# ThibHlln/smartpy

Hardware: AMD Instinct MI355X
Metric: MC sample-timesteps/sec/GPU; 1e5 LHS x hourly 10-yr forcing (higher is better)
Workload: dtype f64

## Files before the change

smartpy_amd/csrc/smart_capi.hip:

```cpp
#include "smart_capi_internal.h"
#include "smart_fast_entry.h"

#include <cmath>
#include <cstdarg>
#include <cstdio>
#include <cstdlib>
#include <cstring>
#include <mutex>
#include <vector>

namespace smart {

static_assert(kStatusSliceTimeout == SMART_STATUS_SLICE_TIMEOUT && kStatusStalePlan == SMART_STATUS_STALE_PLAN,
              "status bits of smart_device.h and include/smart_amd.h");

static thread_local char g_err[512] = "";

int fail(int code, const char *fmt, ...)
{
    va_list ap;
    va_start(ap, fmt);
    vsnprintf(g_err, sizeof(g_err), fmt, ap);
    va_end(ap);
    return code;
}

void clear_error() { g_err[0] = 0; }

int hip_fail(hipError_t e, const char *what) { return fail(SMART_E_NO_DEVICE, "%s: %s", what, hipGetErrorString(e)); }

__global__ __launch_bounds__(256) void smart_obs_prepare(const double *obs, long R, double *ws)
{
    __shared__ double sh[512];
    __shared__ double st[5];
    const long c = blockIdx.x;
    double *w = ws + c * (kWsHead + R);
    obs_stats<true>(obs + c * R, R, st, w + kWsHead, sh);
    const long r1 = first_observed_row(obs + c * R, R, sh);
    if (threadIdx.x < 5)
        w[threadIdx.x] = st[threadIdx.x];
    if (threadIdx.x == 5)
        w[kWsFirst] = (double)r1;
}

__global__ void smart_forcing_scan(KArgs a, const double2 *__restrict__ forcing)
{
    const double2 *__restrict__ f = forcing + (long)blockIdx.y * a.T;
    int bad = 0;
    bool wild = false;
    const unsigned long long top = 0x7ff0000000000000ull;
    for (long t = (long)blockIdx.x * blockDim.x + threadIdx.x; t < a.T; t += (long)gridDim.x * blockDim.x) {
        bad |= forcing_flags_of_step(a, f, t);
        const double2 v = f[t];
        wild = wild || (__builtin_bit_cast(unsigned long long, v.x) & top) == top ||
               (__builtin_bit_cast(unsigned long long, v.y) & top) == top;
    }
    if (a.codes) {
        uint2 *codes = const_cast<uint2 *>(a.codes) + (long)blockIdx.y * code_chunks(a.T);
        for (long ch = (long)blockIdx.x * blockDim.x + threadIdx.x; ch < code_chunks(a.T);
             ch += (long)gridDim.x * blockDim.x) {
            uint2 w = make_uint2(0u, 0u);
            if ((ch + 1) * kChunk <= a.T) {
                const double2 *__restrict__ v = f + ch * kChunk;
                w = chunk_codes(ch, step_kind(v[0]), step_kind(v[1]), step_kind(v[2]), step_kind(v[3]), a.pair_stride);
            }
            codes[ch] = w;
        }
    }
    if (a.estream) {
        double *rec = const_cast<double *>(a.estream) + (long)blockIdx.y * every_pairs(a.T) * 8;
        unsigned *codes = const_cast<unsigned *>(a.ecodes) + (long)blockIdx.y * every_pairs(a.T);
        const double *obs = a.obs ? a.obs + (long)blockIdx.y * a.R : nullptr;
        const double *dev = a.ws ? a.ws + (long)blockIdx.y * (kWsHead + a.R) + kWsHead : nullptr;
        for (long p = (long)blockIdx.x * blockDim.x + threadIdx.x; p < every_pairs(a.T); p += (long)gridDim.x * blockDim.x) {
            double r[8] = {0.0, 0.0, 0.0, 0.0, 0.0, 0.0, 0.0, 0.0};
            unsigned code = 0;
            if (2 * p + 1 < a.T) {
                for (int j = 0; j < 2; ++j) {
                    const long t = 2 * p + j, rr = (t + 1) % a.gap == 0 ? (t + 1) / a.gap - 1 : -1;
                    r[4 * j] = f[t].x;
                    r[4 * j + 1] = f[t].y;
                    r[4 * j + 2] = obs && dev && rr >= 0 && rr < a.R ? obs[rr] : 0.0;
                    r[4 * j + 3] = obs && dev && rr >= 0 && rr < a.R ? dev[rr] : 0.0;
                }
                code = a.gap == 1 ? every_code(p, step_kind(f[2 * p]), step_kind(f[2 * p + 1]))
                                  : gap_code(p, a.gap, step_kind(f[2 * p]), step_kind(f[2 * p + 1]));
            }
            for (int j = 0; j < 8; ++j)
                rec[p * 8 + j] = r[j];
            codes[p] = code;
        }
    }
    if (bad)
        __hip_atomic_fetch_or(a.fflags + blockIdx.y, bad, __ATOMIC_RELAXED, __HIP_MEMORY_SCOPE_AGENT);
    if (wild && a.hdr)
        __hip_atomic_fetch_or(a.hdr + kHdrStatus, kStatusNonFiniteForcing, __ATOMIC_RELAXED, __HIP_MEMORY_SCOPE_AGENT);
}

__global__ void smart_workspace_reset(int *hdr, long n_hdr, int *flags, long n_flags)
{
    const long i = (long)blockIdx.x * blockDim.x + threadIdx.x;
    if (i < n_hdr)
        hdr[i] = 0;
    if (i < n_flags)
        flags[i] = 0;
}

__global__ __launch_bounds__(kWave) void smart_classify_rows(KArgs a)
{
    const int cls = wave_class(a, (long)blockIdx.x, (long)blockIdx.y);
    if (threadIdx.x == 0) {
        __hip_atomic_fetch_or(a.hdr + kHdrPlan, 1 << cls, __ATOMIC_RELAXED, __HIP_MEMORY_SCOPE_AGENT);
        if (cls == 3)
            __hip_atomic_fetch_add(a.hdr + kHdrPlanIllCond, 1, __ATOMIC_RELAXED, __HIP_MEMORY_SCOPE_AGENT);
    }
}

__global__ void smart_classify_forcing(KArgs a, int *hdr)
{
    const long c = (long)blockIdx.x * blockDim.x + threadIdx.x;
    if (c < a.n_catch) {
        const int kind = forcing_kind(a, a.fflags[c]);
        __hip_atomic_fetch_or(hdr + kHdrPlan,
                              kind == kForcingIntervals ? SMART_PLAN_FORCING_PIECEWISE
                                                        : (kind == kForcingRuns ? SMART_PLAN_FORCING_RUNS
                                                                                : SMART_PLAN_FORCING_VARYING),
                              __ATOMIC_RELAXED, __HIP_MEMORY_SCOPE_AGENT);
    }
}

constexpr int kMaxDevices = 64, kMaxTodo = 8, kMaxAux = kMaxTodo - 1;

struct DeviceCtx {
    std::once_flag once;
    int n_simd = 0;
    std::mutex mu;
    hipStream_t aux[kMaxAux] = {};
    hipEvent_t fork = nullptr, join[kMaxAux] = {};
    size_t lds_size[kNumFastKernels][17] = {};
    bool lds_known[kNumFastKernels][17] = {};
};

static DeviceCtx g_dev[kMaxDevices];

static DeviceCtx *device_ctx()
{
    int dev = 0;
    if (hipGetDevice(&dev) != hipSuccess || dev < 0 || dev >= kMaxDevices)
        return nullptr;
    DeviceCtx *d = &g_dev[dev];
    std::call_once(d->once, [d, dev] {
        int cus = 0;
        if (hipDeviceGetAttribute(&cus, hipDeviceAttributeMultiprocessorCount, dev) == hipSuccess && cus > 0)
            d->n_simd = cus * 4;
    });
    return d->n_simd > 0 ? d : nullptr;
}

struct Overrides {
    int pair_blocks = -1;
    int time_slices = 0;
    int illcond_form = SMART_LITERAL_FORM_AUTO;
    int exits = -1;
    long max_polls = kDefaultMaxPolls;
    int drop_slice = 0;
    bool allsteps_fast = false;
};

static Overrides read_overrides()
{
    Overrides o;
    if (const char *v = getenv("SMART_PAIR_BLOCKS"))
        o.pair_blocks = atoi(v) != 0;
    if (const char *v = getenv("SMART_TIME_SLICES"))
        o.time_slices = atoi(v) <= 0 ? 1 : atoi(v);
    if (const char *v = getenv("SMART_ILLCOND_FORM"))
        o.illcond_form = !strcmp(v, "rows")    ? SMART_LITERAL_FORM_ROWS
                         : !strcmp(v, "lanes") ? SMART_LITERAL_FORM_LANES
                                               : SMART_LITERAL_FORM_AUTO;
    if (const char *v = getenv("SMART_EXITS"))
        o.exits = atoi(v) != 0;
    if (const char *v = getenv("SMART_DEBUG_MAX_POLLS"))
        o.max_polls = atol(v) > 0 ? atol(v) : kDefaultMaxPolls;
    if (const char *v = getenv("SMART_DEBUG_DROP_SLICE"))
        o.drop_slice = atoi(v);
    if (const char *v = getenv("SMART_ALLSTEPS_MATH"))
        o.allsteps_fast = !strcmp(v, "fast");
    return o;
}

struct FastKernelInfo {
    const void *handle;
    const char *name;
    int cls;
    bool sliced;
    int waves;
};

static const FastKernelInfo kFastKernels[kNumFastKernels] = {
#define X(id, symbol, cls, sliced, waves) {reinterpret_cast<const void *>(&symbol), #symbol, cls, sliced, waves},
    SMART_FAST_KERNELS(X)
#undef X
};

static size_t lds_for_residency(DeviceCtx *d, FastKernel k, int per_cu)
{
    if (per_cu < 1 || per_cu > 16)
        return 0;
    if (!d->lds_known[k][per_cu]) {
        size_t found = 0;
        for (size_t x = (size_t)(160 * 1024 / per_cu) / 256 * 256;
             x >= 1024 && x > (size_t)(160 * 1024 / (per_cu + 1)) - 2048; x -= 256) {
            int nb = 0;
            if (hipOccupancyMaxActiveBlocksPerMultiprocessor(&nb, kFastKernels[k].handle, kWave, x) != hipSuccess)
                break;
            if (nb == per_cu) {
                found = x;
                break;
            }
            if (nb > per_cu)
                break;
        }
        d->lds_size[k][per_cu] = found;
        d->lds_known[k][per_cu] = true;
    }
    return d->lds_size[k][per_cu];
}

static int merged_report(const SmartEnsemble *e);

extern "C" __attribute__((used, visibility("default"))) volatile char smart_lint_stamp[40] = "SMART_LINT_STAMP=unchecked";

static bool pair_blocks_wanted(const Overrides &ov)
{
    if (ov.pair_blocks >= 0)
        return ov.pair_blocks != 0;
    static const char ok[] = "SMART_LINT_STAMP=pairs-ok";
    for (size_t i = 0; i + 1 < sizeof(ok); ++i)
        if (smart_lint_stamp[i] != ok[i])
            return false;
    return true;
}

static bool uses_records(const SmartEnsemble *e)
{
    const int merged = merged_report(e);
    return merged == kReportEvery || ((merged == kReportMean || merged == kReportLast) && e->report_gap % kChunk != 0);
}

struct Layout {
    size_t header = 0;
    size_t stats_off = 0, stats = 0;
    size_t state_off = 0, state = 0;
    size_t flags_off = 0, flags = 0;
    size_t codes_off = 0, codes = 0;
    size_t ecodes_off = 0;
    size_t total = 0;
    size_t handover() const { return state + flags; }
};

static bool sizes_make_sense(const SmartEnsemble *e)
{
    return e->n_catchments >= 1 && e->n_samples >= 1 && e->n_steps >= 0 && e->report_gap >= 1;
}

static Layout layout(const SmartEnsemble *e, bool sliced)
{
    Layout l;
    const size_t C = (size_t)(e->n_catchments < 1 ? 1 : e->n_catchments);
    l.header = ((size_t)kHdrInts + C) * sizeof(int);
    l.header = (l.header + 255) / 256 * 256;
    if (!sizes_make_sense(e))
        return l;
    l.stats_off = l.header;
    if (e->objfn)
        l.stats = C * (size_t)(kWsHead + smart_n_reports(e->n_steps, e->report_gap, e->report_type)) * sizeof(double);
    l.state_off = l.stats_off + l.stats;
    const size_t blocks = (size_t)((e->n_samples + kWave - 1) / kWave) * C;
    if (sliced) {
        l.state = blocks * kSegFields * kWave * sizeof(double);
        l.flags = (blocks + 1) / 2 * 2 * sizeof(int);
    }
    l.flags_off = l.state_off + l.state;
    l.codes_off = l.ecodes_off = l.flags_off + l.flags;
    const int merged = merged_report(e);
    if (e->math_mode != SMART_MATH_FAST) {
    } else if (uses_records(e)) {
        const size_t records = C * (size_t)every_pairs(e->n_steps) * 8 * sizeof(double);
        l.ecodes_off = l.codes_off + records;
        l.codes = records + C * (size_t)every_pairs(e->n_steps) * sizeof(unsigned);
    } else if (merged == kReportMean || merged == kReportLast) {
        l.codes = C * (size_t)code_chunks(e->n_steps) * sizeof(uint2);
    }
    l.codes = (l.codes + 255) / 256 * 256;
    l.total = l.codes_off + l.codes;
    return l;
}

static int check(const SmartEnsemble *e)
{
    if (!e)
        return fail(SMART_E_NULL, "SmartEnsemble pointer is NULL");
    if (e->n_catchments < 1 || e->n_samples < 1 || e->n_steps < 1 || e->n_warm < 0 || e->report_gap < 1)
        return fail(SMART_E_SIZE, "sizes must satisfy n_catchments, n_samples, n_steps, report_gap >= 1 and n_warm >= 0 "
                                  "(got %lld, %lld, %lld, %lld, %lld)",
                    (long long)e->n_catchments, (long long)e->n_samples, (long long)e->n_steps,
                    (long long)e->report_gap, (long long)e->n_warm);
    if (e->report_type != SMART_REPORT_SUMMARY && e->report_type != SMART_REPORT_RAW)
        return fail(SMART_E_REPORT_TYPE, "Reporting type '%d' unknown.", (int)e->report_type);
    if (e->math_mode != SMART_MATH_LITERAL && e->math_mode != SMART_MATH_FAST)
        return fail(SMART_E_MODE, "math mode '%d' unknown.", (int)e->math_mode);
    if (e->n_warm > e->n_steps)
        return fail(SMART_E_WARMUP, "The warm-up duration (%lld steps) cannot exceed the length of the simulation period "
                                    "(%lld steps) because the beginning of the simulation period is used as made-up "
                                    "warm-up data.",
                    (long long)e->n_warm, (long long)e->n_steps);
    if (e->report_type == SMART_REPORT_SUMMARY && (e->n_steps % e->report_gap || e->n_warm % e->report_gap))
        return fail(SMART_E_GAP, "summary report: simulation length %lld and warm-up length %lld must be multiples of the "
                                 "report gap %lld",
                    (long long)e->n_steps, (long long)e->n_warm, (long long)e->report_gap);
    if (!(e->delta_sec > 0.0))
        return fail(SMART_E_SIZE, "delta_sec must be > 0");
    if (!e->area_m2 || !e->forcing || !e->params || !e->gw)
        return fail(SMART_E_NULL, "area_m2, forcing, params and gw are required");
    if (e->params_catchment_stride != 0 && e->params_catchment_stride < e->n_samples * 10)
        return fail(SMART_E_SIZE, "params_catchment_stride must be 0 or >= n_samples * 10");
    if (e->discharge && e->discharge_ld < e->n_samples)
        return fail(SMART_E_SIZE, "discharge_ld must be >= n_samples");
    if (e->objfn && (!e->obs || !e->workspace))
        return fail(SMART_E_NULL, "objfn needs obs and workspace");
    if (e->objfn && e->workspace_bytes < (int64_t)layout(e, false).state_off)
        return fail(SMART_E_SIZE, "workspace_bytes %lld is less than the %lld the header and the observation statistics need",
                    (long long)e->workspace_bytes, (long long)layout(e, false).state_off);
    if (e->time_slices < 0)
        return fail(SMART_E_SIZE, "time_slices must be >= 0");
    if (e->plan != 0 && !(e->plan & SMART_PLAN_VALID))
        return fail(SMART_E_SIZE, "plan must be 0 or a value returned by smart_plan_ensemble");
    if (e->literal_form < SMART_LITERAL_FORM_AUTO || e->literal_form > SMART_LITERAL_FORM_LANES)
        return fail(SMART_E_MODE, "literal_form must be SMART_LITERAL_FORM_AUTO, _ROWS or _LANES");
    clear_error();
    return SMART_OK;
}

int device_ready()
{
    int n = 0;
    hipError_t err = hipGetDeviceCount(&n);
    if (err != hipSuccess)
        return hip_fail(err, "hipGetDeviceCount");
    if (n < 1)
        return fail(SMART_E_NO_DEVICE, "no HIP device is visible; this engine has no CPU fallback");
    return SMART_OK;
}

static int merged_report(const SmartEnsemble *e)
{
    if (e->report_type == SMART_REPORT_SUMMARY && e->report_gap >= 2)
        return kReportMean;
    if (e->final_vars)
        return -1;
    if (e->report_gap == 1)
        return kReportEvery;
    if (e->report_type == SMART_REPORT_RAW && e->n_steps % e->report_gap == 0 && e->n_warm % e->report_gap == 0)
        return kReportLast;
    return -1;
}

static int plan_time_slices(const SmartEnsemble *e, int n_simd, const Overrides &ov, int *per_simd, double *load)
{
    const long blocks = (e->n_samples + kWave - 1) / kWave * e->n_catchments;
    const long cap = (blocks + n_simd - 1) / n_simd;
    *per_simd = (int)(cap < 1 ? 1 : cap);
    *load = (double)blocks / (double)n_simd;
    if (merged_report(e) < 0)
        return 1;
    const long n_all = e->n_warm / e->report_gap + e->n_steps / e->report_gap;
    const int forced = e->time_slices ? e->time_slices : ov.time_slices;
    if (forced == 1 || n_all < 64)
        return 1;
    if (forced > 1)
        return forced < n_all / 4 ? forced : (int)(n_all / 4);
    if (blocks <= n_simd || blocks > 48L * n_simd)
        return 1;
    const long want = blocks >= 10L * n_simd ? 8 : 24;
    return (int)(n_all / 64 < want ? n_all / 64 : want);
}

static bool device_says_sliced(const SmartEnsemble *e, const Overrides &ov)
{
    if (e->math_mode != SMART_MATH_FAST || !sizes_make_sense(e))
        return false;
    int per_simd = 0, n_dev = 0;
    double load = 0.0;
    DeviceCtx *d = hipGetDeviceCount(&n_dev) == hipSuccess && n_dev > 0 ? device_ctx() : nullptr;
    return d && plan_time_slices(e, d->n_simd, ov, &per_simd, &load) > 1;
}

struct Workspace {
    Layout lay;
    int *hdr = nullptr, *fflags = nullptr;
    double *stats = nullptr;
    char *state = nullptr;
    char *codes = nullptr;
};

static Workspace carve(const SmartEnsemble *e, const Overrides &ov)
{
    Workspace w;
    const Layout &l = w.lay = layout(e, device_says_sliced(e, ov));
    const size_t bytes = e->workspace && e->workspace_bytes > 0 ? (size_t)e->workspace_bytes : 0;
    if (bytes < l.header)
        return w;
    char *base = (char *)e->workspace;
    w.hdr = (int *)base;
    w.fflags = w.hdr + kHdrInts;
    if (l.stats && bytes >= l.state_off)
        w.stats = (double *)(base + l.stats_off);
    if (l.handover() && bytes >= l.codes_off)
        w.state = base + l.state_off;
    if (l.codes && bytes >= l.total)
        w.codes = base + l.codes_off;
    return w;
}

static KArgs kernel_args(const SmartEnsemble *e, const Workspace &w)
{
    KArgs a;
    a.N = e->n_samples;
    a.T = e->n_steps;
    a.W = e->n_warm;
    a.gap = e->report_gap;
    a.R = smart_n_reports(e->n_steps, e->report_gap, e->report_type);
    a.first_len = e->report_type == SMART_REPORT_RAW && e->n_steps % e->report_gap ? e->n_steps % e->report_gap
                                                                                 : e->report_gap;
    a.report_type = e->report_type;
    a.dt = e->delta_sec;
    a.area = e->area_m2;
    a.forcing = e->forcing;
    a.params = e->params;
    a.pstride_c = e->params_catchment_stride;
    a.extra = e->extra;
    a.initial = e->initial;
    a.obs = e->obs;
    a.gw_obs = e->gw_obs;
    a.ws = e->objfn ? w.stats : nullptr;
    a.discharge = e->discharge;
    a.ld = e->discharge_ld;
    a.gw = e->gw;
    a.objfn = e->objfn;
    a.final_vars = e->final_vars;
    a.np_mean = e->math_mode == SMART_MATH_LITERAL && e->report_type == SMART_REPORT_SUMMARY && a.gap >= 8 && a.gap <= 128;
    a.pair_stride = e->final_vars ? (int)kPairStrideSplit : (int)kPairStride;
    a.n_catch = e->n_catchments;
    a.n_blocks = (a.N + kWave - 1) / kWave;
    a.seg_blocks = a.n_blocks * a.n_catch;
    a.hdr = w.hdr;
    a.fflags = nullptr;
    const int merged = merged_report(e);
    if ((merged == kReportMean || merged == kReportLast) && a.gap <= 0x7fffffff) {
        for (long q = 1; q * q <= a.gap && a.n_div < kMaxDiv; ++q)
            if (a.gap % q == 0 && a.gap / q >= 2)
                a.div[a.n_div++] = (int)(a.gap / q);
        for (long q = (long)std::sqrt((double)a.gap) + 1; q >= 2 && a.n_div < kMaxDiv; --q)
            if (q * q < a.gap && a.gap % q == 0 && q < a.div[a.n_div - 1])
                a.div[a.n_div++] = (int)q;
    }
    return a;
}

static void reset_workspace(const Workspace &w, long n_catch, int *flags, long n_flags, hipStream_t s)
{
    const long n_hdr = kHdrInts + n_catch, n = n_hdr > n_flags ? n_hdr : n_flags;
    hipLaunchKernelGGL(smart_workspace_reset, dim3((unsigned)((n + 255) / 256)), dim3(256), 0, s, w.hdr, n_hdr, flags,
                       n_flags);
}

static void set_codes(KArgs *a, const Workspace &w, const Overrides &ov)
{
    a->codes = nullptr, a->estream = nullptr, a->ecodes = nullptr;
    if (!w.codes || !pair_blocks_wanted(ov))
        return;
    if (w.lay.ecodes_off != w.lay.codes_off) {
        a->estream = (const double *)w.codes;
        a->ecodes = (const unsigned *)(w.codes + (w.lay.ecodes_off - w.lay.codes_off));
    } else {
        a->codes = (const uint2 *)w.codes;
    }
}

static void scan_forcing(const SmartEnsemble *e, KArgs a, const Workspace &w, const Overrides &ov, hipStream_t s)
{
    a.fflags = w.fflags;
    set_codes(&a, w, ov);
    hipLaunchKernelGGL(smart_forcing_scan, dim3(64, (unsigned)e->n_catchments), dim3(256), 0, s, a,
                       reinterpret_cast<const double2 *>(e->forcing));
}

static hipError_t launch_kernel(FastKernel k, KArgs a, dim3 grid, size_t lds, hipStream_t s)
{
    const double2 *forcing = reinterpret_cast<const double2 *>(a.forcing);
    const double *obs = a.obs, *ws = a.ws;
    void *args[] = {&a, &forcing, &obs, &ws};
    return hipLaunchKernel(kFastKernels[k].handle, grid, dim3(kWave), args, lds, s);
}

struct Decision {
    FastKernel todo[kMaxTodo];
    int n_todo = 0;
    bool overflow = false;
    void push(FastKernel k)
    {
        if (n_todo < kMaxTodo)
            todo[n_todo++] = k;
        else
            overflow = true;
    }
    int n_seg = 1, per_simd = 0, exits = 0;
    int class_mask = 0, pc_mask = 0;
    int report = -1;
    bool intervals = false;
    double load = 0.0;
    long illcond_blocks = 0;
    bool illcond_rows = true;
};

constexpr int kIllCondRowRounds = 2;

static long count_illcond_blocks(const SmartEnsemble *e, int plan)
{
    const long counted = (plan >> SMART_PLAN_ILLCOND_BLOCKS_SHIFT) & SMART_PLAN_ILLCOND_BLOCKS_MAX;
    const long all = (long)((e->n_samples + kWave - 1) / kWave * e->n_catchments);
    return counted > 0 && counted < SMART_PLAN_ILLCOND_BLOCKS_MAX ? counted : all;
}

static bool illcond_form(const SmartEnsemble *e, int n_simd, long blocks, const Overrides &ov)
{
    const int form = e->literal_form != SMART_LITERAL_FORM_AUTO ? e->literal_form : ov.illcond_form;
    if (form != SMART_LITERAL_FORM_AUTO)
        return form == SMART_LITERAL_FORM_ROWS;
    const long all = (long)((e->n_samples + kWave - 1) / kWave * e->n_catchments);
    return blocks * kIllCondWaves + (all - blocks) <= (long)kIllCondRowRounds * n_simd;
}

static int decide(const SmartEnsemble *e, const DeviceCtx *d, const Workspace &w, const Overrides &ov, Decision *out)
{
    Decision &x = *out;
    x.report = merged_report(e);
    x.intervals = x.report == kReportMean;
    const int plan = (e->plan & SMART_PLAN_VALID) ? e->plan : (0x3f | SMART_PLAN_FORCING_RUNS);
    x.n_seg = plan_time_slices(e, d->n_simd, ov, &x.per_simd, &x.load);
    if (x.n_seg > 1 && !w.state)
        x.n_seg = 1;
    x.exits = ov.exits >= 0 ? ov.exits : x.load > 2.5;
    x.class_mask = plan & 0xf;
    if (plan & SMART_PLAN_CLASS_REGULAR) {
        if (x.intervals) {
            if (plan & SMART_PLAN_FORCING_PIECEWISE) {
                x.push(e->final_vars ? kIntervalsStates : (x.exits ? kIntervalsExits : kIntervals));
                x.pc_mask |= kPcIntervals;
            }
            if (plan & SMART_PLAN_FORCING_RUNS) {
                x.push(e->final_vars ? kRunsStates : (x.exits ? kRunsExits : kRuns));
                x.pc_mask |= kPcRuns;
            }
            if (plan & SMART_PLAN_FORCING_VARYING) {
                x.push(e->final_vars ? kStepsStates : kSteps);
                x.pc_mask |= kPcSteps;
            }
        } else if (x.report == kReportLast) {
            if (plan & SMART_PLAN_FORCING_PIECEWISE) {
                x.push(kIntervalsRaw);
                x.pc_mask |= kPcIntervals;
            }
            if (plan & (SMART_PLAN_FORCING_RUNS | SMART_PLAN_FORCING_VARYING)) {
                x.push(kStepsRaw);
                x.pc_mask |= kPcSteps | kPcRuns;
            }
        } else if (x.report == kReportEvery) {
            x.push(kStepsEvery);
            x.pc_mask = kPcIntervals | kPcSteps | kPcRuns;
        } else {
            x.push(kPlain);
        }
    }
    if (plan & SMART_PLAN_CLASS_STIFF)
        x.push(kStiff);
    if (plan & SMART_PLAN_CLASS_GUARD)
        x.push(kGuard);
    if (plan & SMART_PLAN_CLASS_ILLCOND) {
        x.illcond_blocks = count_illcond_blocks(e, plan);
        x.illcond_rows = illcond_form(e, d->n_simd, x.illcond_blocks, ov);
        x.push(x.illcond_rows ? kIllCond : kIllCondLanes);
    }
    if (x.overflow)
        return fail(SMART_E_SIZE, "internal: a call wants more than %d kernels", kMaxTodo);
    if (x.n_todo == 0)
        return fail(SMART_E_SIZE, "the plan names no class of rows");
    return SMART_OK;
}

static int run(const SmartEnsemble *e, const Overrides &ov, bool literal_rows = false)
{
    int rc = check(e);
    if (rc)
        return rc;
    if ((rc = device_ready()))
        return rc;
    hipStream_t s = (hipStream_t)e->stream;
    const Workspace w = carve(e, ov);
    KArgs a = kernel_args(e, w);

    if (e->objfn)
        hipLaunchKernelGGL(smart_obs_prepare, dim3((unsigned)e->n_catchments), dim3(256), 0, s, e->obs, a.R, w.stats);

    const dim3 grid((unsigned)a.n_blocks, (unsigned)e->n_catchments);
    if (e->math_mode == SMART_MATH_LITERAL) {
        if (w.hdr)
            reset_workspace(w, e->n_catchments, nullptr, 0, s);
        a.hdr = nullptr;
        launch_literal(a, grid, a.np_mean ? (size_t)a.gap * kWave * sizeof(double) : 0, s, literal_rows);
        HIP_TRY(hipGetLastError());
        return SMART_OK;
    }

    DeviceCtx *d = device_ctx();
    if (!d)
        return fail(SMART_E_NO_DEVICE, "cannot query the current HIP device");
    Decision x;
    if ((rc = decide(e, d, w, ov, &x)))
        return rc;
    const int n_seg = x.n_seg, n_todo = x.n_todo;
    a.exits = x.exits;
    a.class_mask = x.class_mask;
    a.pc_mask = x.pc_mask;

    KArgs a_sliced = a;
    if (n_seg > 1) {
        a_sliced.n_seg = n_seg;
        a_sliced.seg_state = (double *)w.state;
        a_sliced.seg_flag = (int *)(w.state + (w.lay.flags_off - w.lay.state_off));
        a_sliced.max_polls = ov.max_polls;
        a_sliced.debug_drop = ov.drop_slice;
    }
    if (w.hdr) {
        reset_workspace(w, e->n_catchments, a_sliced.seg_flag, n_seg > 1 ? a.seg_blocks : 0, s);
        scan_forcing(e, a, w, ov, s);
        if (x.report >= 0 && (x.class_mask & SMART_PLAN_CLASS_REGULAR)) {
            a.fflags = a_sliced.fflags = w.fflags;
            set_codes(&a, w, ov);
            a_sliced.codes = a.codes, a_sliced.estream = a.estream, a_sliced.ecodes = a.ecodes;
        }
    }

    std::lock_guard<std::mutex> lock(d->mu);
    auto launch = [&](FastKernel k, hipStream_t st) -> hipError_t {
        if (kFastKernels[k].sliced && n_seg > 1) {
            const size_t lds = x.per_simd <= 3 ? lds_for_residency(d, k, 4 * x.per_simd) : 0;
            return launch_kernel(k, a_sliced, dim3((unsigned)(a.seg_blocks * n_seg), 1), lds, st);
        }
        return launch_kernel(k, a, dim3(grid.x * kFastKernels[k].waves, grid.y), 0, st);
    };
    if (n_todo == 1) {
        HIP_TRY(launch(x.todo[0], s));
        return SMART_OK;
    }
    if (!d->fork) {
        HIP_TRY(hipEventCreateWithFlags(&d->fork, hipEventDisableTiming));
        for (int i = 0; i < kMaxAux; ++i) {
            HIP_TRY(hipStreamCreateWithFlags(&d->aux[i], hipStreamNonBlocking));
            HIP_TRY(hipEventCreateWithFlags(&d->join[i], hipEventDisableTiming));
        }
    }
    HIP_TRY(hipEventRecord(d->fork, s));
    for (int i = 1; i < n_todo; ++i) {
        HIP_TRY(hipStreamWaitEvent(d->aux[i - 1], d->fork, 0));
        HIP_TRY(launch(x.todo[i], d->aux[i - 1]));
        HIP_TRY(hipEventRecord(d->join[i - 1], d->aux[i - 1]));
    }
    HIP_TRY(launch(x.todo[0], s));
    for (int i = 1; i < n_todo; ++i)
        HIP_TRY(hipStreamWaitEvent(s, d->join[i - 1], 0));
    return SMART_OK;
}

static int describe(const SmartEnsemble *e, const Overrides &ov, char *text, int64_t len)
{
    if (!text || len < 1)
        return fail(SMART_E_NULL, "smart_describe_launch: no room for the text");
    text[0] = 0;
    int rc = check(e);
    if (rc)
        return rc;
    if (e->math_mode == SMART_MATH_LITERAL) {
        snprintf(text, (size_t)len, "smart_ensemble_literal");
        return SMART_OK;
    }
    if ((rc = device_ready()))
        return rc;
    DeviceCtx *d = device_ctx();
    if (!d)
        return fail(SMART_E_NO_DEVICE, "cannot query the current HIP device");
    Decision x;
    if ((rc = decide(e, d, carve(e, ov), ov, &x)))
        return rc;
    const long blocks = (e->n_samples + kWave - 1) / kWave * e->n_catchments;
    size_t used = 0;
    for (int i = 0; i < x.n_todo && used + 1 < (size_t)len; ++i) {
        const FastKernelInfo &k = kFastKernels[x.todo[i]];
        char *at = text + used;
        const size_t room = (size_t)len - used;
        int n;
        if (k.sliced && x.n_seg > 1)
            n = snprintf(at, room, "%s%s[%d slices x %ld blocks, %d resident per SIMD]", i ? " + " : "", k.name, x.n_seg,
                         blocks, x.per_simd);
        else if (k.cls == 3)
            n = snprintf(at, room, "%s%s[%ld of %ld blocks, one sample per %s]", i ? " + " : "", k.name, x.illcond_blocks,
                         blocks, k.waves > 1 ? "DPP row x 16 wavefronts" : "lane");
        else
            n = snprintf(at, room, "%s%s[%ld blocks]", i ? " + " : "", k.name, blocks);
        if (n < 0)
            break;
        used += (size_t)n;
    }
    return SMART_OK;
}

static int64_t workspace_bytes(const SmartEnsemble *e, const Overrides &ov)
{
    return e ? (int64_t)layout(e, device_says_sliced(e, ov)).total : 0;
}

static int make_plan(const SmartEnsemble *e, const Overrides &ov, int32_t *plan)
{
    if (!plan)
        return fail(SMART_E_NULL, "smart_plan_ensemble: plan is NULL");
    *plan = 0;
    int rc = check(e);
    if (rc)
        return rc;
    if ((rc = device_ready()))
        return rc;
    const Workspace w = carve(e, ov);
    if (!w.hdr)
        return fail(SMART_E_NULL, "smart_plan_ensemble needs a workspace of smart_workspace_bytes() bytes");
    hipStream_t s = (hipStream_t)e->stream;
    KArgs a = kernel_args(e, w);
    reset_workspace(w, e->n_catchments, nullptr, 0, s);
    hipLaunchKernelGGL(smart_classify_rows, dim3((unsigned)a.n_blocks, (unsigned)e->n_catchments), dim3(kWave), 0, s, a);
    if (merged_report(e) == kReportMean || merged_report(e) == kReportLast) {
        scan_forcing(e, a, w, ov, s);
        a.fflags = w.fflags;
        hipLaunchKernelGGL(smart_classify_forcing, dim3((unsigned)((e->n_catchments + 255) / 256)), dim3(256), 0, s,
                           a, w.hdr);
    }
    HIP_TRY(hipGetLastError());
    int bits[2] = {0, 0};
    static_assert(kHdrPlanIllCond == kHdrPlan + 1, "read back together");
    HIP_TRY(hipMemcpyAsync(bits, w.hdr + kHdrPlan, sizeof(bits), hipMemcpyDeviceToHost, s));
    HIP_TRY(hipStreamSynchronize(s));
    const long n_ill = bits[1] < 0 ? 0 : (bits[1] > SMART_PLAN_ILLCOND_BLOCKS_MAX ? SMART_PLAN_ILLCOND_BLOCKS_MAX : bits[1]);
    *plan = SMART_PLAN_VALID | (bits[0] & (0x3f | SMART_PLAN_FORCING_RUNS)) |
            (int32_t)(n_ill << SMART_PLAN_ILLCOND_BLOCKS_SHIFT);
    return SMART_OK;
}

static int launch_status(const SmartEnsemble *e, int32_t *status)
{
    if (!e || !status)
        return fail(SMART_E_NULL, "smart_launch_status: NULL argument");
    *status = 0;
    if (!e->workspace || e->workspace_bytes < (int64_t)layout(e, false).header)
        return SMART_OK;
    int rc = device_ready();
    if (rc)
        return rc;
    int word = 0;
    HIP_TRY(hipMemcpyAsync(&word, (const int *)e->workspace + kHdrStatus, sizeof(int), hipMemcpyDeviceToHost,
                           (hipStream_t)e->stream));
    HIP_TRY(hipStreamSynchronize((hipStream_t)e->stream));
    *status = word;
    return SMART_OK;
}

struct HookCache {
    int device = -1;
    double *forcing = nullptr;
    size_t cap = 0;
    std::vector<double> rain, peva;
    double *io = nullptr;
    size_t io_cap = 0;
    std::vector<double> stage;
    int64_t n_calls = 0, n_malloc = 0, bytes_up = 0, n_fast = 0;
    struct Known {
        int64_t len, gap;
        int type, forcing_bits;
// ... 335 lines not shown
```

smartpy_amd/csrc/smart_device.h:

```cpp
#pragma once

#include "smart_matrix_common.h"

#include <hip/hip_runtime.h>

#include <type_traits>

namespace smart {

constexpr int kMaxDiv = 12;
constexpr int kForcingInsane = 1 << 30;

struct KArgs {
    long N, T, W, gap, R, first_len;
    int report_type;
    int np_mean;
    double dt;
    const double *area;
    const double *forcing;
    const double *params;
    long pstride_c;
    const double *extra;
    const double *initial;
    const double *obs;
    const double *gw_obs;
    const double *ws;
    double *discharge;
    long ld;
    double *gw;
    double *objfn;
    double *final_vars;
    int exits = 1;
    int class_mask = 0xf;
    int pc_mask = 0x7;
    int *hdr = nullptr;
    int *fflags = nullptr;
    const double *estream = nullptr;
    const unsigned *ecodes = nullptr;
    int pair_stride = 0;
    const uint2 *codes = nullptr;
    int n_div = 0;
    int div[kMaxDiv] = {};
    int n_seg = 1;
    long n_catch = 1;
    long n_blocks = 0;
    long seg_blocks = 0;
    double *seg_state = nullptr;
    int *seg_flag = nullptr;
    long max_polls = 0;
    int debug_drop = 0;
};

enum SegField : int {
    kSegState = 0,
    kSegDenRaw = 13,
    kSegPend = 15,
    kSegOutflows = 16,
    kSegA = 17,
    kSegB,
    kSegC1,
    kSegC2,
    kSegC3,
    kSegShift,
    kSegFields
};
enum HdrInt : int {
    kHdrStatus = 0,
    kHdrTicket = 1,
    kHdrPlan = 8,
    kHdrPlanIllCond = 9,
    kHdrInts = 64
};
constexpr int kStatusSliceTimeout = 1, kStatusStalePlan = 2, kStatusNonFiniteForcing = 4;

__device__ __forceinline__ void raise_status(const KArgs &a, int bit)
{
    if (a.hdr && threadIdx.x == 0)
        __hip_atomic_fetch_or(a.hdr + kHdrStatus, bit, __ATOMIC_RELAXED, __HIP_MEMORY_SCOPE_AGENT);
}

#define SMART_NOPS_0 ""
#define SMART_NOPS_1 "s_nop 0\n\t"
#define SMART_NOPS_2 SMART_NOPS_1 SMART_NOPS_1
#define SMART_NOPS_4 SMART_NOPS_2 SMART_NOPS_2
#define SMART_NOPS_8 SMART_NOPS_4 SMART_NOPS_4
#define SMART_NOPS_3 SMART_NOPS_2 SMART_NOPS_1
#define SMART_NOPS_5 SMART_NOPS_4 SMART_NOPS_1
#define SMART_NOPS_6 SMART_NOPS_4 SMART_NOPS_2
#define SMART_NOPS_7 SMART_NOPS_4 SMART_NOPS_3
#define SMART_NOPS_9 SMART_NOPS_8 SMART_NOPS_1
#define SMART_NOPS_10 SMART_NOPS_8 SMART_NOPS_2
#define SMART_NOPS_11 SMART_NOPS_8 SMART_NOPS_3
#define SMART_NOPS_12 SMART_NOPS_8 SMART_NOPS_4
#define SMART_NOPS_13 SMART_NOPS_8 SMART_NOPS_5
#define SMART_NOPS_14 SMART_NOPS_8 SMART_NOPS_6
#define SMART_NOPS_15 SMART_NOPS_8 SMART_NOPS_7
#define SMART_NOPS_(n) SMART_NOPS_##n
#define SMART_NOPS(n) SMART_NOPS_(n)
#define SMART_PLACE_LOOP(phase) asm volatile(".p2align 6\n\t" SMART_NOPS(phase))
#ifndef SMART_STEPS_PHASE
#define SMART_STEPS_PHASE 1
#endif
#ifndef SMART_PS_STRIDE
#define SMART_PS_STRIDE 2368
#endif
#ifndef SMART_E_STRIDE
#define SMART_E_STRIDE 2240
#endif
#ifndef SMART_EVERY_PHASE
#define SMART_EVERY_PHASE 2
#endif
#ifndef SMART_P_STRIDE
#define SMART_P_STRIDE 2112
#endif
#ifndef SMART_STEP_ARMS
#define SMART_STEP_ARMS 1
#endif

constexpr int kIllCondWaves = 16;
constexpr int kWsHead = 8;
constexpr int kWsFirst = 5;

__device__ inline void finish_objectives(const double *st, double A, double B, double C1, double C2, double C3,
                                         double gw_sim, double gw_obs, double *o)
{
    const double n = st[0], se = st[2], see = st[3], sd = st[4];
    const double inv_n = 1.0 / n;
    const double m1 = C1 * inv_n;
    const double var_s = C2 * inv_n - m1 * m1;
    const double var_e = see * inv_n;
    const double cov = (C3 - sd * m1) * inv_n;
    double cc = cov / sqrt(var_s * var_e);
    if (!is_nan_bits(cc))
        cc = fmin(fmax(cc, -1.0), 1.0);
    const double alpha = sqrt(var_s / var_e);
    const double beta = 1.0 + A / se;
    o[0] = 1.0 - B / see;
    o[1] = 1.0 - sqrt((cc - 1.0) * (cc - 1.0) + (alpha - 1.0) * (alpha - 1.0) + (beta - 1.0) * (beta - 1.0));
    o[2] = cc;
    o[3] = alpha;
    o[4] = beta;
    o[5] = 100.0 * (A / se);
    o[6] = sqrt(B * inv_n);
    if (!is_nan_bits(gw_obs))
        o[7] = (gw_obs - 0.1 <= gw_sim && gw_sim <= gw_obs + 0.1) ? 1.0 : 0.0;
    else
        o[7] = quiet_nan();
}

__device__ inline double np_pairwise_lds(const double *col, long n)
{
    if (n < 8) {
        double r = 0.0;
        for (long i = 0; i < n; ++i)
            r += col[i * kWave];
        return r;
    }
    double r0 = col[0], r1 = col[kWave], r2 = col[2 * kWave], r3 = col[3 * kWave];
    double r4 = col[4 * kWave], r5 = col[5 * kWave], r6 = col[6 * kWave], r7 = col[7 * kWave];
    long i = 8;
    for (; i < n - (n % 8); i += 8) {
        const double *b = col + i * kWave;
        r0 += b[0];
        r1 += b[kWave];
        r2 += b[2 * kWave];
        r3 += b[3 * kWave];
        r4 += b[4 * kWave];
        r5 += b[5 * kWave];
        r6 += b[6 * kWave];
        r7 += b[7 * kWave];
    }
    double res = ((r0 + r1) + (r2 + r3)) + ((r4 + r5) + (r6 + r7));
    for (; i < n; ++i)
        res += col[i * kWave];
    return res;
}

struct StepGeneric {};
struct StepAllWet {};

__device__ __forceinline__ bool same_bits(double x, double y)
{
    return __builtin_bit_cast(long long, x) == __builtin_bit_cast(long long, y);
}

constexpr int kChunk = 4;

template <class Model, class = void>
struct chunk_hook : std::false_type {};
template <class Model>
struct chunk_hook<Model, std::enable_if_t<Model::kChunkHook>> : std::true_type {};

template <class Model, class = void>
struct chunk_modes : std::false_type {};
template <class Model>
struct chunk_modes<Model, std::enable_if_t<Model::kChunkModes>> : std::true_type {};

template <class Model, class Body, class ChunkEnd>
__device__ __forceinline__ void time_loop_chunked(const Model &m, const double2 *__restrict__ f, long n, Body &&body,
                                                  ChunkEnd &&chunk_end)
{
    const long n_chunks = n / kChunk;
    double2 cur[kChunk], nxt[kChunk];
    if (n_chunks > 0) {
// ... 721 lines not shown

template <class Body>
__device__ __forceinline__ void interval_loop(const double2 *__restrict__ f, long i0, long i1, long gap, Body &&body)
{
    interval_walk<false>(f, nullptr, nullptr, i0, i1, gap, 0,
                         [&](int k, const double2 v, double, double, auto) { body(k, v); });
}

template <class Body>
__device__ __forceinline__ void interval_loop_obs(const double2 *__restrict__ f, const double *obs, const double *dev,
                                                  long i0, long i1, long gap, int lead, Body &&body)
{
    interval_walk<true>(f, obs + i0, dev + i0, i0, i1, gap, lead, body);
}

constexpr int kPollSleep = 100;
constexpr long kDefaultMaxPolls = 1000000;

struct Work {
    long block, c;
    int seg;
};

__device__ __forceinline__ Work claim_work(const KArgs &a, int sliced_kernel)
{
    Work w;
    if (a.n_seg > 1) {
        unsigned t = 0;
        if (threadIdx.x == 0)
            t = __hip_atomic_fetch_add(reinterpret_cast<unsigned *>(a.hdr) + kHdrTicket + sliced_kernel, 1u,
                                       __ATOMIC_RELAXED, __HIP_MEMORY_SCOPE_AGENT);
        t = (unsigned)__builtin_amdgcn_readfirstlane((int)t);
        const long slot = (long)(t % (unsigned long)a.seg_blocks);
        w.seg = (int)(t / (unsigned long)a.seg_blocks);
        w.c = slot / a.n_blocks;
        w.block = slot % a.n_blocks;
    } else {
        w.block = blockIdx.x;
        w.c = blockIdx.y;
        w.seg = 0;
    }
    return w;
}

__device__ __forceinline__ bool wait_for_slice(const KArgs &a, long slot, int seg)
{
    int *flag = a.seg_flag + slot;
    long polls = 0;
    int v;
    while ((v = __hip_atomic_load(flag, __ATOMIC_RELAXED, __HIP_MEMORY_SCOPE_AGENT)) > -seg && v < seg) {
        __builtin_amdgcn_s_sleep(kPollSleep);
        if (++polls > a.max_polls) {
            raise_status(a, kStatusSliceTimeout);
            return false;
        }
    }
    __builtin_amdgcn_fence(__ATOMIC_ACQUIRE, "agent");
    return v >= seg;
}

__device__ __forceinline__ void publish_slice(const KArgs &a, long slot, int seg, bool good)
{
    asm volatile("s_waitcnt vmcnt(0)" ::: "memory");
    __builtin_amdgcn_fence(__ATOMIC_RELEASE, "agent");
    asm volatile("s_waitcnt vmcnt(0)" ::: "memory");
    if (threadIdx.x == 0)
        __hip_atomic_store(a.seg_flag + slot, good ? seg + 1 : -(seg + 1), __ATOMIC_RELAXED, __HIP_MEMORY_SCOPE_AGENT);
}

constexpr int kReportMean = 0, kReportLast = 1, kReportEvery = 2;

template <class Model, int FORCING, int REPORT = kReportMean>
__device__ __forceinline__ void run_ensemble_merged(const KArgs &a, const double2 *__restrict__ forcing,
                                                    const double *__restrict__ obs_all,
                                                    const double *__restrict__ ws_all, long block, long catchment,
                                                    int seg, int fflags)
{
    constexpr bool piecewise = FORCING != kForcingVarying;
    constexpr bool runs = FORCING == kForcingRuns;
    static_assert(REPORT == kReportMean || (!Model::kSplit && !runs), "raw / every-step reports: merged model, no runs");
    static_assert(REPORT != kReportEvery || !piecewise, "a report every step is a step loop");
    static_assert(Model::kStateFields <= kSegPend, "the model's states end in front of the other hand-over fields");
    const LaneCtx x = lane_ctx(a, block, catchment);
    const long slot = catchment * a.n_blocks + block;
    Model m;
    init_model(a, x, m);
    const long gap = a.gap;
    const long run_len = runs ? run_length(a, fflags) : gap;
    if constexpr (piecewise)
        m.setup_intervals(REPORT == kReportLast ? run_len - 1 : run_len);
    const double2 *__restrict__ f = forcing + x.c * a.T;

    int fits = 0;
    unsigned not_quick = ~0u;
    if constexpr (piecewise && Model::kWetAsm) {
        m.note_capacity();
        const bool fits_b = m.over_mask == 0;
        fits = __builtin_amdgcn_readfirstlane((int)fits_b);
        not_quick = 0u - (unsigned)__builtin_amdgcn_readfirstlane((int)!(fits_b && !(fflags & kForcingInsane)));
        asm("" : "+s"(fits), "+s"(not_quick));
    }
    auto no_bits = [](double x, unsigned unless = 0) {
        unsigned long long b = __builtin_bit_cast(unsigned long long, x) | unless;
        asm("" : "+s"(b));
        return b == 0;
    };
    auto interval = [&](const double2 v, double &acc, double &num, double &den) {
        if constexpr (piecewise && Model::kWetAsm) {
            if (no_bits(v.x, not_quick)) {
                if (no_bits(v.y)) {
                    m.calm_interval(run_len, acc);
                } else {
                    m.dry_interval(-v.y, run_len, acc);
                }
                return;
            }
        }
        const double ex = m.excess(v.x, v.y);
        if (ex < 0.0) {
            m.dry_interval(ex, run_len, acc);
        } else {
            if constexpr (piecewise && Model::kWetAsm)
                m.wet_interval(ex, run_len, acc, num, den, fits);
            else
                m.wet_interval(ex, run_len, acc, num, den);
        }
    };

    [[maybe_unused]] auto interval_last = [&](const double2 v, double &qo, double &qg, double &qi) {
        if constexpr (piecewise && REPORT == kReportLast && Model::kWetAsm) {
            double sink = 0.0, n0 = 0.0, n1 = 0.0;
            if (no_bits(v.x, not_quick)) {
                if (no_bits(v.y)) {
                    m.calm_interval(gap - 1, sink);
                    m.last_step_flows(qo, qg, qi);
                    m.calm_interval(1, sink);
                } else {
                    m.dry_interval_last(-v.y, gap, qo, qg, qi);
                }
                return;
            }
            const double ex = m.excess(v.x, v.y);
            if (ex < 0.0) {
                m.dry_interval_last(ex, gap, qo, qg, qi);
            } else {
                m.wet_interval(ex, gap - 1, sink, n0, n1, fits);
                m.last_step_flows(qo, qg, qi);
                m.wet_interval(ex, 1, sink, n0, n1, fits);
            }
        }
    };

    const long n_warm = a.W / gap, n_all = n_warm + a.R;
    const long g0 = n_all * seg / a.n_seg, g1 = n_all * (seg + 1) / a.n_seg;
    const long wa = g0 < n_warm ? g0 : n_warm, wb = g1 < n_warm ? g1 : n_warm;
    const long ra = g0 > n_warm ? g0 - n_warm : 0, rb = g1 > n_warm ? g1 - n_warm : 0;
    const bool last = seg == a.n_seg - 1;

    Reporter rep;
    rep.init(a, x, obs_all, ws_all);
    [[maybe_unused]] const double *__restrict__ obs_c = obs_all ? obs_all + x.c * a.R : nullptr;
    [[maybe_unused]] const double *__restrict__ dev_c = ws_all ? ws_all + x.c * (kWsHead + a.R) + kWsHead : nullptr;
    [[maybe_unused]] const uint2 *codes_c = a.codes ? a.codes + x.c * code_chunks(a.T) : nullptr;
    [[maybe_unused]] const double2 *f_asm = reinterpret_cast<const double2 *>(a.forcing) + x.c * a.T;
    double num = 0.0, den = 0.0, q_out_total = 0.0;
    [[maybe_unused]] double num_raw = 0.0, den_raw = 0.0;
    double *hand = a.seg_state + (slot * kSegFields) * kWave + x.lane;
    if (seg > 0) {
        if (!wait_for_slice(a, slot, seg)) {
            const double nan = quiet_nan();
            if (a.discharge && x.live)
                for (long r = ra; r < rb; ++r)
                    a.discharge[(x.c * a.R + r) * a.ld + x.n] = nan;
            if (last) {
                if (x.live) {
                    a.gw[x.c * a.N + x.n] = nan;
                    if (a.objfn)
                        for (int i = 0; i < 8; ++i)
                            a.objfn[(x.c * a.N + x.n) * 8 + i] = nan;
                    if (a.final_vars)
                        for (int i = 0; i < 19; ++i)
                            a.final_vars[(x.c * a.N + x.n) * 19 + i] = nan;
                }
            } else {
                publish_slice(a, slot, seg, false);
            }
            return;
        }
        m.load_state(hand, kWave);
        if constexpr (REPORT == kReportLast) {
            num_raw = hand[kSegOutflows * kWave];
            den_raw = hand[kSegDenRaw * kWave];
        } else {
            q_out_total = hand[kSegOutflows * kWave];
        }
        rep.A = hand[kSegA * kWave];
        rep.B = hand[kSegB * kWave];
        rep.C1 = hand[kSegC1 * kWave];
        rep.C2 = hand[kSegC2 * kWave];
        rep.C3 = hand[kSegC3 * kWave];
        rep.shift = hand[kSegShift * kWave];
    }

    double *const park = Model::kSplit ? a.final_vars + (x.c * a.N + x.n) * 19 : nullptr;
    auto park_state = [&]() {
        if constexpr (Model::kSplit) {
            m.save_state(park, 1);
            if constexpr (!piecewise)
                park[15] = m.pend;
        }
    };

    double s0 = 0.0, s1 = 0.0, s2 = 0.0;
    const double inv_gap = 1.0 / (double)gap;
    const bool starts_run = ra == 0 && (rb > 0 || last);
    constexpr bool deferring = !piecewise;
    [[maybe_unused]] const int n_lead = (int)(rep.r1 + 1 > ra ? (rep.r1 + 1 < rb ? rep.r1 + 1 - ra : rb - ra) : 0);
    [[maybe_unused]] int store = __builtin_amdgcn_readfirstlane((int)(a.discharge != nullptr));
    asm("" : "+s"(store));
    [[maybe_unused]] const int k_park = Model::kSplit && ra <= a.R - 1 && a.R - 1 < rb ? (int)(a.R - 1 - ra) : -1;
    if constexpr (piecewise)
        rep.begin_rows(a, x, ra);
    if constexpr (runs) {
        const long per = gap / run_len;
        interval_loop(f, wa * per, wb * per, run_len, [&](int, const double2 v) { interval(v, s0, s1, s2); });
        if (starts_run)
            m.begin_run();
        long j = 0, r = ra;
        double acc = 0.0;
        rep.prime(a, ra);
        interval_loop(f, ra * per, rb * per, run_len, [&](int, const double2 v) {
            if (Model::kSplit && j == 0 && r == a.R - 1)
                park_state();
            interval(v, acc, num, den);
            if (++j == per) {
                rep.emit_ahead(a, x, r, acc * inv_gap);
                q_out_total += acc;
                acc = 0.0;
                j = 0;
                ++r;
            }
        });
    } else if constexpr (piecewise && REPORT == kReportLast) {
        interval_loop(f, wa, wb, gap, [&](int, const double2 v) { interval_last(v, s0, s1, s2); });
        if (starts_run)
            m.begin_run();
        if (rep.want_obj) {
            interval_loop_obs(f, rep.obs, rep.ws + kWsHead, ra, rb, gap, n_lead,
                              [&](int k, const double2 v, const double e, const double w, auto lead_tag) {
                                  double qo, qg, qi;
                                  interval_last(v, qo, qg, qi);
                                  rep.template emit_interval<true, decltype(lead_tag)::value, false>(
                                      store, a.ld, rep.sets_shift(ra + k), qo, e, w);
                                  num_raw += qg;
                                  den_raw += qi;
                              });
        } else {
            interval_loop(f, ra, rb, gap, [&](int, const double2 v) {
                double qo, qg, qi;
                interval_last(v, qo, qg, qi);
                rep.template emit_interval<false, false, true>(store, a.ld, false, qo, 0.0, 0.0);
                num_raw += qg;
                den_raw += qi;
            });
        }
    } else if constexpr (piecewise) {
        interval_loop(f, wa, wb, gap, [&](int, const double2 v) { interval(v, s0, s1, s2); });
        if (starts_run)
            m.begin_run();
        if (rep.want_obj) {
            interval_loop_obs(f, rep.obs, rep.ws + kWsHead, ra, rb, gap, n_lead,
                              [&](int k, const double2 v, const double e, const double w, auto lead_tag) {
                                  if (Model::kSplit && k == k_park)
                                      park_state();
                                  double acc = 0.0;
                                  interval(v, acc, num, den);
                                  rep.template emit_interval<true, decltype(lead_tag)::value, false>(
                                      store, a.ld, rep.sets_shift(ra + k), acc * inv_gap, e, w);
                                  q_out_total += acc;
                              });
        } else {
            interval_loop(f, ra, rb, gap, [&](int k, const double2 v) {
                if (Model::kSplit && k == k_park)
                    park_state();
                double acc = 0.0;
                interval(v, acc, num, den);
                rep.template emit_interval<false, false, true>(store, a.ld, false, acc * inv_gap, 0.0, 0.0);
                q_out_total += acc;
            });
        }
    } else {
        m.begin_lazy(seg > 0 ? hand[kSegPend * kWave] : 0.0);
        long k = 0, r = ra;
        (void)k;
        double acc = 0.0;
        auto report = [&]() __attribute__((always_inline)) {
            auto emit = [&](const double val) __attribute__((always_inline)) {
                rep.emit(a, x, r, val);
                rep.next_row(a);
            };
            if constexpr (REPORT == kReportMean) {
                emit(acc * inv_gap);
                ++r;
                k = 0;
                q_out_total += acc;
                acc = 0.0;
                if (Model::kSplit && r == a.R - 1)
                    park_state();
            } else if constexpr (REPORT == kReportLast) {
                emit(acc);
                ++r;
                num_raw += m.q_gw;
                den_raw += m.q_in;
            }
        };
        [[maybe_unused]] double *row = a.discharge ? a.discharge + (x.c * a.R + ra) * a.ld : nullptr;
        [[maybe_unused]] auto report_every = [&](auto store_tag, auto obs_tag, const double e, const double w) {
            const double val = acc;
            if constexpr (decltype(store_tag)::value) {
                if (x.live)
                    row[x.n] = val;
                row += a.ld;
            }
            if (decltype(obs_tag)::value && !is_missing_mark(w))
                rep.add_moments(val, e, w);
            q_out_total += val;
        };
#if SMART_STEP_ARMS
        const bool quick = m.zero_ok && !(fflags & kForcingInsane);
        auto walk = [&](auto quick_tag) __attribute__((always_inline)) {
            constexpr bool Q = decltype(quick_tag)::value;
#pragma nounroll
            for (int stretch = 0; stretch < 2; ++stretch) {
                const long i0 = stretch ? ra : wa, i1 = stretch ? rb : wb;
                if (stretch == 1) {
                    rep.begin_rows(a, x, ra);
                    acc = 0.0;
                    if (starts_run)
                        m.begin_run();
                    if (Model::kSplit && ra == a.R - 1 && rb > ra)
                        park_state();
// ... 204 lines not shown
```

smartpy_amd/csrc/smart_fast_entry.h:

```cpp
#pragma once

#include "smart_fast_model.h"

namespace smart {

#define SMART_FAST_KERNELS(X)                                                                                          \
    X(kIntervalsExits, smart_fast_intervals_exits, 0, true, 1)                                                         \
    X(kIntervals, smart_fast_intervals, 0, true, 1)                                                                    \
    X(kIntervalsStates, smart_fast_intervals_states, 0, true, 1)                                                       \
    X(kSteps, smart_fast_steps, 0, true, 1)                                                                            \
    X(kStepsStates, smart_fast_steps_states, 0, true, 1)                                                               \
    X(kPlain, smart_fast_plain, 0, false, 1)                                                                           \
    X(kStiff, smart_fast_stiff, 1, false, 1)                                                                           \
    X(kGuard, smart_fast_guard, 2, false, 1)                                                                           \
    X(kIllCond, smart_fast_illcond, 3, false, kIllCondWaves)                                                           \
    X(kRunsExits, smart_fast_runs_exits, 0, true, 1)                                                                   \
    X(kRuns, smart_fast_runs, 0, true, 1)                                                                              \
    X(kRunsStates, smart_fast_runs_states, 0, true, 1)                                                                 \
    X(kStepsRaw, smart_fast_steps_raw, 0, true, 1)                                                                     \
    X(kIntervalsRaw, smart_fast_intervals_raw, 0, true, 1)                                                             \
    X(kStepsEvery, smart_fast_steps_every, 0, true, 1)                                                                 \
    X(kIllCondLanes, smart_fast_illcond_lanes, 3, false, 1)

#define SMART_FAST_KERNEL(name)                                                                                        \
    __global__ __launch_bounds__(kWave) void name(KArgs a, const double2 *__restrict__ forcing,                        \
                                                  const double *__restrict__ obs, const double *__restrict__ ws)

enum FastKernel : int {
#define X(id, symbol, cls, sliced, waves) id,
    SMART_FAST_KERNELS(X)
#undef X
    kNumFastKernels
};

#define X(id, symbol, cls, sliced, waves) SMART_FAST_KERNEL(symbol);
SMART_FAST_KERNELS(X)
#undef X

constexpr int kTicketIntervals = 0, kTicketSteps = 1, kTicketRuns = 2, kTicketStepsRaw = 3, kTicketIntervalsRaw = 4,
              kTicketEvery = 5;
static_assert(kHdrTicket + kTicketEvery < kHdrPlan, "the tickets end in front of the plan word of smart_plan_ensemble");

template <int CLS>
__device__ __forceinline__ bool block_is_mine(const KArgs &a, const Work &w)
{
    const int cls = wave_class(a, w.block, w.c);
    if (cls == CLS)
        return true;
    if (w.seg == 0 && !((a.class_mask >> cls) & 1))
        raise_status(a, kStatusStalePlan);
    return false;
}

template <int FORCING>
__device__ __forceinline__ bool forcing_is_mine(const KArgs &a, int fflags, const Work &w)
{
    const int kind = forcing_kind(a, fflags);
    if (kind == FORCING)
        return true;
    if (w.seg == 0 && !(a.pc_mask & pc_bit(kind)))
        raise_status(a, kStatusStalePlan);
    return false;
}

template <class Model, int FORCING, int REPORT = kReportMean>
__device__ __forceinline__ void merged_kernel(const KArgs &a, const double2 *__restrict__ forcing,
                                              const double *__restrict__ obs, const double *__restrict__ ws)
{
    constexpr int ticket = REPORT == kReportEvery  ? kTicketEvery
                           : REPORT == kReportLast ? (FORCING == kForcingIntervals ? kTicketIntervalsRaw : kTicketStepsRaw)
                           : FORCING == kForcingIntervals ? kTicketIntervals
                                                          : (FORCING == kForcingVarying ? kTicketSteps : kTicketRuns);
    const Work w = claim_work(a, ticket);
    if (!block_is_mine<0>(a, w))
        return;
    const int fflags = forcing_flags(a, forcing, w.c);
    if constexpr (REPORT == kReportLast && FORCING == kForcingVarying) {
        if (forcing_kind(a, fflags) == kForcingIntervals) {
            if (w.seg == 0 && !(a.pc_mask & kPcIntervals))
                raise_status(a, kStatusStalePlan);
            return;
        }
    } else if constexpr (REPORT != kReportEvery) {
        if (!forcing_is_mine<FORCING>(a, fflags, w))
            return;
    }
    run_ensemble_merged<Model, FORCING, REPORT>(a, forcing, obs, ws, w.block, w.c, w.seg, fflags);
}

}
```

Baseline: 918.5 billion.

## Taper time-slice lengths so trailing slices shrink and the sequential handover tail shortens

Replaces the uniform split of report intervals across time slices with a tapered split. Early slices get equal units and the last few (up to six) get progressively shorter lengths. Slices are chained through a state handover, so shorter final slices are meant to cut the serial tail after the earlier slices finish. The taper is on by default when enough slices and steps exist, can be turned off with an environment variable, and comes with an optional compile-time timeline instrumentation. The risk is extra per-slice overhead and uneven work if the slice handover pattern differs from what the taper assumes.

```diff
diff --git a/smartpy_amd/csrc/smart_capi.hip b/smartpy_amd/csrc/smart_capi.hip
--- a/smartpy_amd/csrc/smart_capi.hip
+++ b/smartpy_amd/csrc/smart_capi.hip
@@ -161,6 +161,7 @@
     int pair_blocks = -1;
     int time_slices = 0;
     int illcond_form = SMART_LITERAL_FORM_AUTO;
+    bool taper = true;
     int exits = -1;
     long max_polls = kDefaultMaxPolls;
     int drop_slice = 0;
@@ -174,6 +175,8 @@
         o.pair_blocks = atoi(v) != 0;
     if (const char *v = getenv("SMART_TIME_SLICES"))
         o.time_slices = atoi(v) <= 0 ? 1 : atoi(v);
+    if (const char *v = getenv("SMART_SLICE_TAPER"))
+        o.taper = atoi(v) != 0;
     if (const char *v = getenv("SMART_ILLCOND_FORM"))
         o.illcond_form = !strcmp(v, "rows")    ? SMART_LITERAL_FORM_ROWS
                          : !strcmp(v, "lanes") ? SMART_LITERAL_FORM_LANES
@@ -255,6 +258,9 @@
     size_t flags_off = 0, flags = 0;
     size_t codes_off = 0, codes = 0;
     size_t ecodes_off = 0;
+#ifdef SMART_SLICE_TIMELINE
+    size_t timeline_off = 0, timeline = 0;
+#endif
     size_t total = 0;
     size_t handover() const { return state + flags; }
 };
@@ -294,6 +300,12 @@
     }
     l.codes = (l.codes + 255) / 256 * 256;
     l.total = l.codes_off + l.codes;
+#ifdef SMART_SLICE_TIMELINE
+    l.timeline_off = l.total;
+    if (sliced)
+        l.timeline = blocks * kTimelineSlices * kTimelineFields * sizeof(unsigned long long);
+    l.total += l.timeline;
+#endif
     return l;
 }
 
@@ -402,6 +414,9 @@
     double *stats = nullptr;
     char *state = nullptr;
     char *codes = nullptr;
+#ifdef SMART_SLICE_TIMELINE
+    char *timeline = nullptr;
+#endif
 };
 
 static Workspace carve(const SmartEnsemble *e, const Overrides &ov)
@@ -420,6 +435,10 @@
         w.state = base + l.state_off;
     if (l.codes && bytes >= l.total)
         w.codes = base + l.codes_off;
+#ifdef SMART_SLICE_TIMELINE
+    if (l.timeline && bytes >= l.total)
+        w.timeline = base + l.timeline_off;
+#endif
     return w;
 }
 
@@ -637,10 +656,14 @@
     KArgs a_sliced = a;
     if (n_seg > 1) {
         a_sliced.n_seg = n_seg;
+        a_sliced.taper = ov.taper && slice_taper_applies(a.W / a.gap + a.R, n_seg);
         a_sliced.seg_state = (double *)w.state;
         a_sliced.seg_flag = (int *)(w.state + (w.lay.flags_off - w.lay.state_off));
         a_sliced.max_polls = ov.max_polls;
         a_sliced.debug_drop = ov.drop_slice;
+#ifdef SMART_SLICE_TIMELINE
+        a_sliced.timeline = (unsigned long long *)w.timeline;
+#endif
     }
     if (w.hdr) {
         reset_workspace(w, e->n_catchments, a_sliced.seg_flag, n_seg > 1 ? a.seg_blocks : 0, s);
diff --git a/smartpy_amd/csrc/smart_device.h b/smartpy_amd/csrc/smart_device.h
--- a/smartpy_amd/csrc/smart_device.h
+++ b/smartpy_amd/csrc/smart_device.h
@@ -1,5 +1,6 @@
 #pragma once
 
+#include "smart_slice_cuts.h"
 #include "smart_matrix_common.h"
 
 #include <hip/hip_runtime.h>
@@ -42,6 +43,7 @@
     int n_div = 0;
     int div[kMaxDiv] = {};
     int n_seg = 1;
+    int taper = 0;
     long n_catch = 1;
     long n_blocks = 0;
     long seg_blocks = 0;
@@ -49,7 +51,19 @@
     int *seg_flag = nullptr;
     long max_polls = 0;
     int debug_drop = 0;
+#ifdef SMART_SLICE_TIMELINE
+    unsigned long long *timeline = nullptr;
+#endif
 };
+#ifdef SMART_SLICE_TIMELINE
+constexpr int kTimelineFields = 5, kTimelineSlices = 64;
+__device__ __forceinline__ void timeline_note(const KArgs &a, long block, long c, int seg, int field,
+                                              unsigned long long value)
+{
+    if (a.timeline && a.n_seg > 1 && seg < kTimelineSlices && seg < a.n_seg && threadIdx.x == 0)
+        a.timeline[((long)seg * a.seg_blocks + c * a.n_blocks + block) * kTimelineFields + field] = value;
+}
+#endif
 
 enum SegField : int {
     kSegState = 0,
@@ -1077,7 +1091,8 @@
     };
 
     const long n_warm = a.W / gap, n_all = n_warm + a.R;
-    const long g0 = n_all * seg / a.n_seg, g1 = n_all * (seg + 1) / a.n_seg;
+    const long g0 = a.taper ? slice_cut_tapered(n_all, seg, a.n_seg) : n_all * seg / a.n_seg;
+    const long g1 = a.taper ? slice_cut_tapered(n_all, seg + 1, a.n_seg) : n_all * (seg + 1) / a.n_seg;
     const long wa = g0 < n_warm ? g0 : n_warm, wb = g1 < n_warm ? g1 : n_warm;
     const long ra = g0 > n_warm ? g0 - n_warm : 0, rb = g1 > n_warm ? g1 - n_warm : 0;
     const bool last = seg == a.n_seg - 1;
@@ -1112,6 +1127,9 @@
             }
             return;
         }
+#ifdef SMART_SLICE_TIMELINE
+        timeline_note(a, block, catchment, seg, 3, __builtin_amdgcn_s_memrealtime());
+#endif
         m.load_state(hand, kWave);
         if constexpr (REPORT == kReportLast) {
             num_raw = hand[kSegOutflows * kWave];
diff --git a/smartpy_amd/csrc/smart_fast_entry.h b/smartpy_amd/csrc/smart_fast_entry.h
--- a/smartpy_amd/csrc/smart_fast_entry.h
+++ b/smartpy_amd/csrc/smart_fast_entry.h
@@ -85,7 +85,17 @@
         if (!forcing_is_mine<FORCING>(a, fflags, w))
             return;
     }
+#ifdef SMART_SLICE_TIMELINE
+    timeline_note(a, w.block, w.c, w.seg, 0, (unsigned long long)(w.seg * a.seg_blocks + w.c * a.n_blocks + w.block));
+    timeline_note(a, w.block, w.c, w.seg, 1,
+                  (unsigned long long)__builtin_amdgcn_s_getreg(63492)
+                      | (unsigned long long)__builtin_amdgcn_s_getreg(63508) << 32);
+    timeline_note(a, w.block, w.c, w.seg, 2, __builtin_amdgcn_s_memrealtime());
+#endif
     run_ensemble_merged<Model, FORCING, REPORT>(a, forcing, obs, ws, w.block, w.c, w.seg, fflags);
+#ifdef SMART_SLICE_TIMELINE
+    timeline_note(a, w.block, w.c, w.seg, 4, __builtin_amdgcn_s_memrealtime());
+#endif
 }
 
 }
diff --git a/smartpy_amd/csrc/smart_slice_cuts.h b/smartpy_amd/csrc/smart_slice_cuts.h
--- /dev/null
+++ b/smartpy_amd/csrc/smart_slice_cuts.h
@@ -0,0 +1,55 @@
+#pragma once
+
+#if defined(__HIPCC__) || defined(__CUDACC__)
+#define SMART_CUTS_FN __host__ __device__ constexpr
+#else
+#define SMART_CUTS_FN constexpr
+#endif
+
+namespace smart {
+
+constexpr long kCutUnit = 1024;
+constexpr int kCutTail = 6;
+constexpr int kCutMinSlices = 8;
+constexpr long kCutMinLen = 4;
+
+SMART_CUTS_FN long cut_tail_sum(int j)
+{
+    return j <= 0 ? 0 : j == 1 ? 614 : j == 2 ? 983 : j == 3 ? 1204 : j == 4 ? 1337 : j == 5 ? 1417 : 1465;
+}
+
+SMART_CUTS_FN int cut_tail_len(long n_seg)
+{
+    const long m = n_seg / 4;
+    return (int)(m < kCutTail ? m : kCutTail);
+}
+
+SMART_CUTS_FN long slice_cut_tapered(long n_all, long k, long n_seg)
+{
+    const int m = cut_tail_len(n_seg);
+    const long n_early = n_seg - m;
+    const long total = n_early * kCutUnit + cut_tail_sum(m);
+    const long upto = k <= n_early ? k * kCutUnit : n_early * kCutUnit + cut_tail_sum((int)(k - n_early));
+    return k >= n_seg ? n_all : n_all * upto / total;
+}
+
+SMART_CUTS_FN bool slice_taper_applies(long n_all, long n_seg)
+{
+    if (n_seg < kCutMinSlices || n_all < n_seg * kCutMinLen)
+        return false;
+    const int m = cut_tail_len(n_seg);
+    const long total = (n_seg - m) * kCutUnit + cut_tail_sum(m);
+    if (n_all * kCutUnit / total < kCutMinLen)
+        return false;
+    for (long k = n_seg - m; k < n_seg; ++k)
+        if (slice_cut_tapered(n_all, k + 1, n_seg) - slice_cut_tapered(n_all, k, n_seg) < kCutMinLen)
+            return false;
+    return 2 * (n_all - slice_cut_tapered(n_all, n_seg - 1, n_seg)) <= slice_cut_tapered(n_all, 1, n_seg);
+}
+
+SMART_CUTS_FN long slice_cut(long n_all, long k, long n_seg, int taper)
+{
+    return taper && slice_taper_applies(n_all, n_seg) ? slice_cut_tapered(n_all, k, n_seg) : n_all * k / n_seg;
+}
+
+}
```

Result: faster. 952.4 billion (median of 6 runs) (+3.7%).
